# chrischoy/DeepGlobalRegistration

Hardware: AMD Instinct MI355X
Metric: pair registrations/sec (FCGF x2 + 1-NN + 6-D inlier net + gate + weighted Procrustes + SE(3) refinement) (higher is better)
Workload: dtype f32 results via 2 x f16 split operands (3 f16 MFMA products per MAC, f32 accumulate); k = 1 convs, kNN re-evaluation and registration in exact f32, SVD in f64

## Files before the change

### deepglobalregistration_amd/csrc/ctx.hip

```cpp
#include <stdarg.h>
#include <time.h>
#include <string.h>

#include "dgr_internal.h"

static thread_local char g_err[1024] = "";

void dgr_set_error(const char *fmt, ...) {
  va_list ap;
  va_start(ap, fmt);
  vsnprintf(g_err, sizeof(g_err), fmt, ap);
  va_end(ap);
}

extern "C" const char *dgr_last_error(void) { return g_err; }
extern "C" const char *dgr_version(void) { return "dgr_hip 0.4 (gfx950)"; }

static constexpr size_t kAlign = 256;
static constexpr size_t kMinChunk = (size_t)256 << 20;

void *DgrArena::alloc(size_t bytes) {
  bytes = (bytes + kAlign - 1) / kAlign * kAlign;
  if (bytes == 0) bytes = kAlign;
  while (cur < chunks.size()) {
    if (offset + bytes <= chunks[cur].size) {
      void *p = chunks[cur].base + offset;
      offset += bytes;
      used_total += bytes;
      if (used_total > high_water) high_water = used_total;
      return p;
    }
    ++cur;
    offset = 0;
  }
  size_t sz = bytes > kMinChunk ? bytes : kMinChunk;
  size_t have = reserved();
  if (sz < have / 2) sz = have / 2;
  char *base = nullptr;
  hipError_t e = hipMalloc((void **)&base, sz);
  if (e != hipSuccess) {
    dgr_set_error("workspace hipMalloc(%zu MiB) failed: %s", sz >> 20, hipGetErrorString(e));
    return nullptr;
  }
  chunks.push_back({base, sz});
  cur = chunks.size() - 1;
  offset = bytes;
  used_total += bytes;
  if (used_total > high_water) high_water = used_total;
  return base;
}

size_t DgrArena::reserved() const {
  size_t s = 0;
  for (auto &c : chunks) s += c.size;
  return s;
}

int DgrArena::reset() {
  if (chunks.size() > 1) {
    DGR_HIP_CHECK(hipDeviceSynchronize());
    for (auto &c : chunks) DGR_HIP_CHECK(hipFree(c.base));
    chunks.clear();
    size_t want = high_water + high_water / 8 + kAlign;
    char *base = nullptr;
    hipError_t e = hipMalloc((void **)&base, want);
    if (e != hipSuccess) {
      dgr_set_error("workspace hipMalloc(%zu MiB) failed: %s", want >> 20, hipGetErrorString(e));
      return DGR_ENOMEM;
    }
    chunks.push_back({base, want});
  }
  cur = 0;
  offset = 0;
  used_total = 0;
  ++generation;
  return DGR_OK;
}

void DgrArena::release() {
  for (auto &c : chunks) (void)hipFree(c.base);
  chunks.clear();
  cur = offset = 0;
}

hipEvent_t DgrEventPool::next() {
  if (used == ev.size()) {
    hipEvent_t e;
    if (hipEventCreate(&e) != hipSuccess) {
      dgr_set_error("hipEventCreate failed");
      return nullptr;
    }
    ev.push_back(e);
  }
  return ev[used++];
// ... 181 lines not shown
```

### deepglobalregistration_amd/csrc/knn.hip

```cpp
#include "knn_prefilter.h"

template <int C, int QPT>
__global__ void __launch_bounds__(KNN_THREADS)
    knn1_kernel(const float *__restrict__ F0, const float *__restrict__ F1, KnnBatch B, int splits,
                u64 *__restrict__ best, const int32_t *run_flag, const int32_t *__restrict__ qlist,
                const int32_t *qcount, int64_t q_begin) {
  __shared__ __attribute__((aligned(16))) float tile[KNN_TB * C];
  const KnnPair d = B.p[blockIdx.z];
  if (run_flag && run_flag[blockIdx.z] == 0) return;
  F0 += d.q0 * C;
  F1 += d.r0 * C;
  best += d.q0;
  const int64_t N0 = d.n0, N1 = d.n1;
  if (qlist) qlist += d.q0 - q_begin;
  const int64_t n_q = qlist ? (int64_t)qcount[blockIdx.z] : N0;
  if ((int64_t)blockIdx.x * KNN_THREADS * QPT >= n_q) return;
  const int64_t q0 = ((int64_t)blockIdx.x * KNN_THREADS + threadIdx.x) * QPT;
  const int rows_per_split = (int)(((N1 + splits - 1) / splits + KNN_TB - 1) / KNN_TB) * KNN_TB;
  const int64_t j_begin = (int64_t)blockIdx.y * rows_per_split;
  const int64_t j_end = min(N1, j_begin + rows_per_split);
  if (j_begin >= j_end) return;
  float q[QPT][C];
  int64_t qrow[QPT];
#pragma unroll
  for (int u = 0; u < QPT; ++u) {
    const int64_t li = min(q0 + u, n_q - 1);
    const int64_t r = qlist ? (int64_t)qlist[li] : li;
    qrow[u] = r;
#pragma unroll
    for (int c = 0; c < C; c += 4) {
      const float4 v = *reinterpret_cast<const float4 *>(F0 + r * C + c);
      q[u][c] = v.x; q[u][c + 1] = v.y; q[u][c + 2] = v.z; q[u][c + 3] = v.w;
    }
  }
  float bd[QPT];
  int bi[QPT];
#pragma unroll
  for (int u = 0; u < QPT; ++u) { bd[u] = __builtin_inff(); bi[u] = 0x7fffffff; }

  for (int64_t j0 = j_begin; j0 < j_end; j0 += KNN_TB) {
    const int nrows = (int)min((int64_t)KNN_TB, j_end - j0);
    __syncthreads();
    for (int e = threadIdx.x; e < KNN_TB * C / 4; e += KNN_THREADS) {
      const int row = e / (C / 4);
      float4 v = make_float4(0.f, 0.f, 0.f, 0.f);
      if (row < nrows) v = *reinterpret_cast<const float4 *>(F1 + (j0 + row) * C + (e % (C / 4)) * 4);
      *reinterpret_cast<float4 *>(tile + e * 4) = v;
    }
    __syncthreads();
    for (int jj = 0; jj < nrows; ++jj) {
      float d0[QPT], d1[QPT];
#pragma unroll
      for (int u = 0; u < QPT; ++u) { d0[u] = 0.f; d1[u] = 0.f; }
#pragma unroll
      for (int c = 0; c < C; c += 4) {
        const float4 b = *reinterpret_cast<const float4 *>(tile + jj * C + c);
#pragma unroll
        for (int u = 0; u < QPT; ++u) {
          const float e0 = q[u][c] - b.x, e1 = q[u][c + 1] - b.y;
          const float e2 = q[u][c + 2] - b.z, e3 = q[u][c + 3] - b.w;
          d0[u] = fmaf(e0, e0, d0[u]);
          d1[u] = fmaf(e1, e1, d1[u]);
          d0[u] = fmaf(e2, e2, d0[u]);
          d1[u] = fmaf(e3, e3, d1[u]);
        }
      }
#pragma unroll
      for (int u = 0; u < QPT; ++u) {
        const float d = d0[u] + d1[u];
        if (d < bd[u]) { bd[u] = d; bi[u] = (int)(j0 + jj); }
      }
    }
  }
#pragma unroll
  for (int u = 0; u < QPT; ++u) {
    if (q0 + u < n_q && bi[u] != 0x7fffffff)
      atomicMin(best + qrow[u], knn_key(bd[u], bi[u] + (int)d.r0));
  }
}

__global__ void knn1_finish(const u64 *__restrict__ best, KnnBatch B, int squared,
                            int64_t *__restrict__ idx_out, float *__restrict__ dist_out) {
  const KnnPair d = B.p[blockIdx.y];
  const int64_t li = (int64_t)blockIdx.x * blockDim.x + threadIdx.x;
  if (li >= d.n0) return;
  const int64_t i = d.q0 + li;
  const u64 k = best[i];
  idx_out[i] = (k == KNN_KEY_NONE) ? d.r0 : (int64_t)(k & 0xffffffffull);
  if (dist_out) {
    const float d2 = __uint_as_float((unsigned int)(k >> 32));
    dist_out[i] = squared ? d2 : sqrtf(d2 + 1e-7f);
  }
}

template <int C>
static int knn_launch(dgr_ctx *ctx, const float *F0, const float *F1, const KnnBatch &B, u64 *best,
                      const int32_t *run_flag, hipStream_t stream, const int32_t *qlist = nullptr,
                      const int32_t *qcount = nullptr, int64_t q_begin = 0) {
  constexpr int QPT = (C <= 32) ? 4 : 2;
  const dim3 grid = knn_brute_grid(ctx, B, QPT, INT32_MAX);
  knn1_kernel<C, QPT><<<grid, KNN_THREADS, 0, stream>>>(F0, F1, B, (int)grid.y, best, run_flag, qlist, qcount, q_begin);
  DGR_LAUNCH_CHECK();
  return DGR_OK;
}


__global__ void __launch_bounds__(256)
    knn_exact_kernel(const float *__restrict__ F0, const float *__restrict__ F1, const int32_t *__restrict__ cand,
                     const int32_t *__restrict__ cand_cnt, int64_t q_begin, int64_t q_end, u64 *__restrict__ best) {
  const int64_t q = q_begin + (int64_t)blockIdx.x * blockDim.x + threadIdx.x;
  if (q >= q_end) return;
  const int cnt = min(cand_cnt[q - q_begin], KNN_SLOTS);
  if (cnt <= 0) return;
  float a[32];
  knn_load_row<32>(a, F0 + q * 32);
  u64 key = KNN_KEY_NONE;
  for (int slot = 0; slot < cnt; ++slot) {
    const int i = cand[(q - q_begin) * KNN_SLOTS + slot];
    const float d = knn_d2<32>(a, F1 + (int64_t)i * 32);
    if (d < __builtin_inff()) {
      const u64 k2 = knn_key(d, i);
      key = k2 < key ? k2 : key;
    }
  }
  if (key != KNN_KEY_NONE) atomicMin(best + q, key);
}

__global__ void knn_overflow_list(const int32_t *__restrict__ cand_cnt, KnnBatch B, int slots, int64_t q_begin,
                                  int32_t *__restrict__ qlist, int32_t *qcount) {
  const KnnPair d = B.p[blockIdx.y];
  const int64_t q = (int64_t)blockIdx.x * blockDim.x + threadIdx.x;
  if (q < d.n0 && cand_cnt[d.q0 - q_begin + q] > slots)
    qlist[d.q0 - q_begin + atomicAdd(qcount + blockIdx.y, 1)] = (int32_t)q;
}
int knn_list_overflows(const KnnBatch &B, const KnnPlan &P, int slots, hipStream_t stream) {
  dim3 grid((unsigned)dgr_ceil_div(P.n0_max, 256), B.np);
  knn_overflow_list<<<grid, 256, 0, stream>>>(P.cand_cnt, B, slots, P.q_begin, P.qlist, P.qcount);
  DGR_LAUNCH_CHECK();
  return DGR_OK;
}

constexpr int KNN_SCAN_MAX = 64, KNN_SCAN_SPLITS = 16;
__global__ void __launch_bounds__(256)
    knn_query_scan_kernel(const float *__restrict__ F0, const float *__restrict__ F1, KnnBatch B, int64_t q_begin,
                          const int32_t *__restrict__ qlist, const int32_t *__restrict__ qcount,
                          u64 *__restrict__ best) {
  __shared__ u64 wkey[4];
  const KnnPair d = B.p[blockIdx.y];
  const int n_q = qcount[blockIdx.y];
  if (n_q <= 0 || n_q > KNN_SCAN_MAX) return;
  const int per = (d.n1 + KNN_SCAN_SPLITS - 1) / KNN_SCAN_SPLITS;
  const int j_begin = blockIdx.x * per, j_end = min(d.n1, j_begin + per);
  for (int li = 0; li < n_q; ++li) {
    const int64_t q = d.q0 + qlist[d.q0 - q_begin + li];
    float a[32];
    knn_load_row<32>(a, F0 + q * 32);
    u64 key = KNN_KEY_NONE;
    for (int j = j_begin + (int)threadIdx.x; j < j_end; j += 256) {
      const float dd = knn_d2<32>(a, F1 + (d.r0 + j) * 32);
      if (dd < __builtin_inff()) {
        const u64 k2 = knn_key(dd, j + (int)d.r0);
        key = k2 < key ? k2 : key;
      }
    }
#pragma unroll
    for (int s2 = 32; s2 > 0; s2 >>= 1) {
      const u64 o = __shfl_xor(key, s2, 64);
      key = o < key ? o : key;
    }
    if ((threadIdx.x & 63) == 0) wkey[threadIdx.x >> 6] = key;
    __syncthreads();
    if (threadIdx.x == 0) {
      u64 k3 = wkey[0];
      for (int w = 1; w < 4; ++w) k3 = wkey[w] < k3 ? wkey[w] : k3;
      if (k3 != KNN_KEY_NONE) atomicMin(best + q, k3);
    }
    __syncthreads();
  }
}

__global__ void knn_long_list_flags(const int32_t *__restrict__ qcount, int np, int32_t *__restrict__ flags) {
  if ((int)threadIdx.x < np) flags[threadIdx.x] = qcount[threadIdx.x] > KNN_SCAN_MAX;
}

static int knn_prefiltered(dgr_ctx *ctx, const float *F0, const float *F1, KnnBatch B, u64 *best, hipStream_t stream) {
  KnnPlan P;
  DGR_CHECK(knn_prefilter_setup<false>(ctx, F0, F1, B, KNN_SLOTS, stream, &P));
  DGR_CHECK((knn_mfma_launch<false, false>(ctx, B, P, KNN_SUB, KNN_SLOTS, stream)));
  DGR_CHECK((knn_mfma_launch<true, false>(ctx, B, P, 1, KNN_SLOTS, stream)));
  knn_exact_kernel<<<(int)dgr_ceil_div(P.span, 256), 256, 0, stream>>>(F0, F1, P.cand, P.cand_cnt, P.q_begin,
                                                                      P.q_begin + P.span, best);
  DGR_LAUNCH_CHECK();
  DGR_CHECK(knn_list_overflows(B, P, KNN_SLOTS, stream));
  dim3 grid(KNN_SCAN_SPLITS, B.np);
  knn_query_scan_kernel<<<grid, 256, 0, stream>>>(F0, F1, B, P.q_begin, P.qlist, P.qcount, best);
  knn_long_list_flags<<<1, 64, 0, stream>>>(P.qcount, B.np, P.flags);
  DGR_LAUNCH_CHECK();
  DGR_CHECK(knn_launch<32>(ctx, F0, F1, B, best, P.flags, stream, P.qlist, P.qcount, P.q_begin));
  return knn_launch<32>(ctx, F0, F1, B, best, P.fallback, stream);
}

int dgr_knn1_batch_impl(dgr_ctx *ctx, const float *F0, const int64_t *off0, const float *F1, const int64_t *off1,
                        int npairs, int C, int squared, int64_t *idx_out, float *dist_out, hipStream_t stream) {
  return knn_for_each_table(ctx, off0, off1, npairs, 1, true, stream, [&](const KnnBatch &B, u64 *best) -> int {
    DGR_CHECK(knn_dispatch(
        B, C,
        [&](auto width, const KnnBatch &pairs) {
          return knn_launch<decltype(width)::value>(ctx, F0, F1, pairs, best, nullptr, stream);
        },
        [&](const KnnBatch &pairs) { return knn_prefiltered(ctx, F0, F1, pairs, best, stream); }));
    dim3 grid((unsigned)dgr_ceil_div(knn_n0_max(B), 256), B.np);
    knn1_finish<<<grid, 256, 0, stream>>>(best, B, squared, idx_out, dist_out);
    DGR_LAUNCH_CHECK();
    return DGR_OK;
  });
}

int dgr_knn1_impl(dgr_ctx *ctx, const float *F0, int64_t N0, const float *F1, int64_t N1, int C,
                  int squared, int64_t *idx_out, float *dist_out, hipStream_t stream) {
  const int64_t off0[2] = {0, N0}, off1[2] = {0, N1};
  return dgr_knn1_batch_impl(ctx, F0, off0, F1, off1, 1, C, squared, idx_out, dist_out, stream);
}

extern "C" int dgr_knn1_l2(dgr_ctx *ctx, const float *F0, int64_t N0, const float *F1, int64_t N1, int C,
                           int squared, int64_t *idx_out, float *dist_out, dgr_stream stream) {
  const int64_t off0[2] = {0, N0}, off1[2] = {0, N1};
  DGR_CHECK(knn_enter("dgr_knn1_l2", ctx, F0, F1, idx_out, off0, off1, 1));
  return dgr_knn1_impl(ctx, F0, N0, F1, N1, C, squared, idx_out, dist_out, (hipStream_t)stream);
}

extern "C" int dgr_knn1_l2_batch(dgr_ctx *ctx, const float *F0, const int64_t *off0, const float *F1,
                                 const int64_t *off1, int npairs, int C, int squared, int64_t *idx_out,
                                 float *dist_out, dgr_stream stream) {
  DGR_CHECK(knn_enter("dgr_knn1_l2_batch", ctx, F0, F1, idx_out, off0, off1, npairs));
  return dgr_knn1_batch_impl(ctx, F0, off0, F1, off1, npairs, C, squared, idx_out, dist_out, (hipStream_t)stream);
}
```

### deepglobalregistration_amd/csrc/knn_prefilter.h

```cpp
#pragma once
#include "knn_common.h"

typedef __attribute__((ext_vector_type(8))) short bf16x8;
typedef __attribute__((ext_vector_type(16))) float f32x16_t;
constexpr float KNN_TAU_C = 8e-5f;
constexpr int KNN_ST = 4;
constexpr int KNN_SLOTS = 32;
#ifndef DGR_KNN_SUB
#define DGR_KNN_SUB 2
#endif
constexpr int KNN_SUB = DGR_KNN_SUB;

__device__ __forceinline__ unsigned short knn_f2bf(float x) {
  uint32_t u = __float_as_uint(x);
  if ((u & 0x7f800000u) == 0x7f800000u) return (unsigned short)((u >> 16) | ((u & 0xffffu) ? 0x40u : 0u));
  u += 0x7fffu + ((u >> 16) & 1u);
  return (unsigned short)(u >> 16);
}
__device__ __forceinline__ float knn_bf2f(unsigned short h) { return __uint_as_float((uint32_t)h << 16); }
__device__ __forceinline__ uint32_t knn_ord(float f) {
  const uint32_t u = __float_as_uint(f);
  return u ^ ((u >> 31) ? 0xffffffffu : 0x80000000u);
}
__device__ __forceinline__ float knn_unord(uint32_t k) {
  return __uint_as_float(k ^ ((k >> 31) ? 0x80000000u : 0xffffffffu));
}
__device__ __forceinline__ int knn_acc_slot(int e, int h) { return (e & 3) + 8 * (e >> 2) + 4 * h; }

template <bool TOPK>
__device__ __forceinline__ int64_t knn_slot_row(int s, int t, int n_tiles) {
  return (int64_t)(TOPK ? (s + t) & 31 : s) * n_tiles + t;
}
template <bool TOPK>
__global__ void __launch_bounds__(256)
    knn_pack_kernel(const float *__restrict__ F0, const float *__restrict__ F1, KnnBatch B,
                    bf16x8 *__restrict__ Qp, bf16x8 *__restrict__ Rp, float *__restrict__ na, float *__restrict__ nb,
                    uint32_t *__restrict__ nb_max, int32_t *__restrict__ fallback) {
  const int pair = blockIdx.y >> 1, side = blockIdx.y & 1;
  const KnnPair d = B.p[pair];
  const int64_t N = side ? d.n1 : d.n0;
  const int64_t n_pad = (N + 31) / 32 * 32;
  const int64_t t = (int64_t)blockIdx.x * blockDim.x + threadIdx.x;
  int64_t row = t >> 2;
  if (row >= n_pad) return;
  const float *F = side ? F1 + d.r0 * 32 : F0 + d.q0 * 32;
  const float scale = side ? -2.f : 1.f;
  const int64_t prow = row;
  if (side) row = knn_slot_row<TOPK>((int)(prow & 31), (int)(prow >> 5), (int)(n_pad >> 5));
  bf16x8 *packed = side ? Rp + (int64_t)d.rt0 * 256 : Qp + (int64_t)d.qb0 * 256;
  float *norms = side ? nb + (int64_t)d.rt0 * 32 : na + (int64_t)d.qb0 * 32;
  const int g = (int)(t & 1), ch = (int)((t >> 1) & 1);
  bf16x8 hi, lo;
#pragma unroll
  for (int e = 0; e < 8; ++e) { hi[e] = 0; lo[e] = 0; }
  if (row < N) {
    const float *src = F + row * 32 + 16 * ch + 8 * g;
    const float4 v0 = *reinterpret_cast<const float4 *>(src), v1 = *reinterpret_cast<const float4 *>(src + 4);
    const float x[8] = {v0.x, v0.y, v0.z, v0.w, v1.x, v1.y, v1.z, v1.w};
#pragma unroll
    for (int e = 0; e < 8; ++e) {
      if (!(fabsf(x[e]) < 1e18f)) fallback[pair] = 1;
      const unsigned short h = knn_f2bf(x[e]);
      const unsigned short l = knn_f2bf(x[e] - knn_bf2f(h));
      hi[e] = (short)knn_f2bf(knn_bf2f(h) * scale);
      lo[e] = (short)knn_f2bf(knn_bf2f(l) * scale);
    }
  }
  const int64_t tile = prow >> 5;
  const int r = (int)(prow & 31);
  packed[(tile * 4 + ch) * 64 + r + 32 * g] = hi;
  packed[(tile * 4 + 2 + ch) * 64 + r + 32 * g] = lo;
  float n = 0.f;
  if (row < N) {
    const float *src = F + row * 32 + 16 * ch + 8 * g;
#pragma unroll
    for (int e = 0; e < 8; ++e) n = fmaf(src[e], src[e], n);
  }
  n += __shfl_xor(n, 1, 64);
  n += __shfl_xor(n, 2, 64);
  if (g == 0 && ch == 0) {
    if (row >= N) n = side ? __builtin_inff() : 0.f;
    else if (side) atomicMax(nb_max + pair, __float_as_uint(n));
    norms[prow] = n;
  }
}

template <bool PASS2, bool TOPK>
__global__ void __launch_bounds__(256, 2)
    knn_mfma_kernel(const bf16x8 *__restrict__ Qp, const bf16x8 *__restrict__ Rp, const float *__restrict__ nbp,
                    KnnBatch B, int splits, int sub_arg, int64_t q_begin, int64_t span, uint32_t *__restrict__ mt,
                    const float *__restrict__ nap, const uint32_t *__restrict__ nb_max,
                    const float *__restrict__ thr_q, int32_t *__restrict__ cand, int32_t *__restrict__ cand_cnt,
                    int slots_arg) {
  __shared__ bf16x8 sA[2][KNN_ST * 4 * 64];
  __shared__ __attribute__((aligned(16))) float sNb[2][KNN_ST * 32];
  const int sub = TOPK ? sub_arg : KNN_SUB, slots = TOPK ? slots_arg : KNN_SLOTS;
  constexpr int NM = TOPK ? 16 : 1;
  const KnnPair d = B.p[blockIdx.z];
  const int n_qblocks = (d.n0 + 31) >> 5, n_rtiles = (d.n1 + 31) >> 5;
  if ((int)blockIdx.x * 16 >= n_qblocks) return;
  const int64_t N0 = d.n0, N1 = d.n1;
  const bf16x8 *Q = Qp + (int64_t)d.qb0 * 256, *R = Rp + (int64_t)d.rt0 * 256;
  const float *nb = nbp + (int64_t)d.rt0 * 32;
  const int64_t qrow0 = d.q0 - q_begin;
  mt += qrow0;
  cand += qrow0 * slots;
  cand_cnt += qrow0;
  const int tid = threadIdx.x;
  const int lane = tid & 63;
  const int wave = __builtin_amdgcn_readfirstlane(tid >> 6);
  const int h = lane >> 5;
  const int qb0 = (blockIdx.x * 4 + wave) * 4;
  bf16x8 bq[4][4];
  float m[4][NM], thr[4];
#pragma unroll
  for (int u = 0; u < 4; ++u) {
    const int qb = min(qb0 + u, n_qblocks - 1);
#pragma unroll
    for (int f = 0; f < 4; ++f) bq[u][f] = Q[((int64_t)qb * 4 + f) * 64 + lane];
#pragma unroll
    for (int e = 0; e < NM; ++e) m[u][e] = __builtin_inff();
    thr[u] = 0.f;
    if constexpr (PASS2) {
      const int64_t q = (int64_t)qb * 32 + (lane & 31);
      const bool live = q < N0 && qb0 + u < n_qblocks;
      if constexpr (TOPK) {
        thr[u] = live ? thr_q[qrow0 + q] : -__builtin_inff();
      } else {
        const float nmax = __uint_as_float(nb_max[blockIdx.z]);
        thr[u] = live ? knn_unord(mt[q]) + KNN_TAU_C * (nap[(int64_t)d.qb0 * 32 + q] + nmax) : -__builtin_inff();
      }
    }
  }
  const int n_stages = (n_rtiles + KNN_ST - 1) / KNN_ST;
  const int sps = (n_stages + splits - 1) / splits;
  const int s_begin = blockIdx.y * sps, s_end = min(n_stages, s_begin + sps);
  const int step = PASS2 ? 1 : sub;
  const int s_first = PASS2 ? s_begin : s_begin + min((int)(blockIdx.y % sub), max(s_end - s_begin - 1, 0));
  if (s_first >= s_end) return;
  bf16x8 pre[KNN_ST];
  float pre_nb = 0.f;
  auto request = [&](int t0) {
#pragma unroll
    for (int j = 0; j < KNN_ST; ++j) pre[j] = R[(int64_t)min(t0 + j, n_rtiles - 1) * 256 + tid];
    if (tid < KNN_ST * 32) pre_nb = nb[(int64_t)min(t0 + (tid >> 5), n_rtiles - 1) * 32 + (tid & 31)];
  };
  auto deposit = [&](int buf) {
#pragma unroll
    for (int j = 0; j < KNN_ST; ++j) sA[buf][j * 256 + tid] = pre[j];
    if (tid < KNN_ST * 32) sNb[buf][tid] = pre_nb;
  };
  request(s_first * KNN_ST);
  deposit(0);
  __syncthreads();
  int buf = 0;
  for (int st = s_first; st < s_end; st += step) {
    const int t0 = st * KNN_ST;
    if (st + step < s_end) request((st + step) * KNN_ST);
#pragma unroll
    for (int j = 0; j < KNN_ST; ++j) {
      const int t = t0 + j;
      if (t >= n_rtiles) break;
      const bf16x8 a0 = sA[buf][(j * 4 + 0) * 64 + lane], a1 = sA[buf][(j * 4 + 1) * 64 + lane];
      const bf16x8 a2 = sA[buf][(j * 4 + 2) * 64 + lane], a3 = sA[buf][(j * 4 + 3) * 64 + lane];
      f32x16_t c0;
#pragma unroll
      for (int g = 0; g < 4; ++g) {
        const float4 v = *reinterpret_cast<const float4 *>(&sNb[buf][j * 32 + 8 * g + 4 * h]);
        c0[4 * g] = v.x; c0[4 * g + 1] = v.y; c0[4 * g + 2] = v.z; c0[4 * g + 3] = v.w;
      }
      f32x16_t acc[4];
#pragma unroll
      for (int u = 0; u < 4; ++u) acc[u] = __builtin_amdgcn_mfma_f32_32x32x16_bf16(a0, bq[u][0], c0, 0, 0, 0);
#pragma unroll
      for (int u = 0; u < 4; ++u) acc[u] = __builtin_amdgcn_mfma_f32_32x32x16_bf16(a1, bq[u][1], acc[u], 0, 0, 0);
#pragma unroll
      for (int u = 0; u < 4; ++u) acc[u] = __builtin_amdgcn_mfma_f32_32x32x16_bf16(a0, bq[u][2], acc[u], 0, 0, 0);
#pragma unroll
      for (int u = 0; u < 4; ++u) acc[u] = __builtin_amdgcn_mfma_f32_32x32x16_bf16(a1, bq[u][3], acc[u], 0, 0, 0);
#pragma unroll
      for (int u = 0; u < 4; ++u) acc[u] = __builtin_amdgcn_mfma_f32_32x32x16_bf16(a2, bq[u][0], acc[u], 0, 0, 0);
#pragma unroll
      for (int u = 0; u < 4; ++u) acc[u] = __builtin_amdgcn_mfma_f32_32x32x16_bf16(a3, bq[u][1], acc[u], 0, 0, 0);
#pragma unroll
      for (int u = 0; u < 4; ++u) {
        if constexpr (!PASS2 && TOPK) {
#pragma unroll
          for (int e = 0; e < 16; ++e) m[u][e] = fminf(m[u][e], acc[u][e]);
        } else {
          float bm = fminf(fminf(acc[u][0], acc[u][1]), fminf(acc[u][2], acc[u][3]));
#pragma unroll
          for (int e = 4; e < 16; e += 4)
            bm = fminf(bm, fminf(fminf(acc[u][e], acc[u][e + 1]), fminf(acc[u][e + 2], acc[u][e + 3])));
          if constexpr (!PASS2) {
            m[u][0] = fminf(m[u][0], bm);
          } else if (!(bm > thr[u])) {
            const int64_t q = (int64_t)(qb0 + u) * 32 + (lane & 31);
#pragma unroll
            for (int e = 0; e < 16; ++e) {
              const int64_t i = knn_slot_row<TOPK>(knn_acc_slot(e, h), t, n_rtiles);
              if (!(acc[u][e] > thr[u]) && q < N0 && i < N1 && qb0 + u < n_qblocks) {
                const int slot = atomicAdd(cand_cnt + q, 1);
                if (slot < slots) cand[q * slots + slot] = (int32_t)(i + d.r0);
              }
            }
          }
        }
      }
    }
    if (st + step < s_end) deposit(buf ^ 1);
    __syncthreads();
    buf ^= 1;
  }
  if constexpr (!PASS2) {
#pragma unroll
    for (int u = 0; u < 4; ++u) {
      const int64_t q = (int64_t)(qb0 + u) * 32 + (lane & 31);
      const bool live = qb0 + u < n_qblocks && q < N0;
      if constexpr (TOPK) {
        if (live) {
#pragma unroll
          for (int e = 0; e < 16; ++e)
            atomicMin(mt + (int64_t)knn_acc_slot(e, h) * span + q, knn_ord(m[u][e]));
        }
      } else {
        const float mm = fminf(m[u][0], __shfl_xor(m[u][0], 32, 64));
        if (lane < 32 && live) atomicMin(mt + q, knn_ord(mm));
      }
    }
  }
}

struct KnnPlan {
  int64_t q_begin, span, n0_max;
  int qb_max, rt_max;
  int qgroups_all;
  bf16x8 *Qp, *Rp;
  float *na, *nb;
  uint32_t *mt;
  float *thr;
  int32_t *qlist, *cand_cnt, *cand;
  uint32_t *nb_max;
  int32_t *fallback, *qcount, *flags;
};

template <bool TOPK>
inline int knn_prefilter_setup(dgr_ctx *ctx, const float *F0, const float *F1, KnnBatch &B, int slots,
                               hipStream_t stream, KnnPlan *plan) {
  KnnPlan &P = *plan;
  DgrArena &arena = ctx->arena;
  int n_qb = 0, n_rt = 0;
  P.qb_max = P.rt_max = P.qgroups_all = 0;
  for (int p = 0; p < B.np; ++p) {
    KnnPair &d = B.p[p];
    d.qb0 = n_qb;
    d.rt0 = n_rt;
    const int qb = (d.n0 + 31) / 32, rt = (d.n1 + 31) / 32;
    n_qb += qb;
    n_rt += rt;
    P.qb_max = std::max(P.qb_max, qb);
    P.rt_max = std::max(P.rt_max, rt);
    P.qgroups_all += (int)dgr_ceil_div(qb, 16);
  }
  P.n0_max = knn_n0_max(B);
  P.span = knn_query_span(B, &P.q_begin);
  const int64_t n_mt = (TOPK ? 32 : 1) * P.span;
  DGR_ALLOC(P.Qp, arena, bf16x8, (int64_t)n_qb * 256);
  DGR_ALLOC(P.Rp, arena, bf16x8, (int64_t)n_rt * 256);
  DGR_ALLOC(P.na, arena, float, (int64_t)n_qb * 32);
  DGR_ALLOC(P.nb, arena, float, (int64_t)n_rt * 32);
  DGR_ALLOC(P.mt, arena, uint32_t, n_mt);
  P.thr = nullptr;
  if (TOPK) DGR_ALLOC(P.thr, arena, float, P.span);
  DGR_ALLOC(P.qlist, arena, int32_t, P.span);
  DGR_ALLOC(P.cand_cnt, arena, int32_t, P.span + 4 * KNN_MAXP);
  DGR_ALLOC(P.cand, arena, int32_t, P.span * slots);
  int32_t *pair_words = P.cand_cnt + P.span;
  P.nb_max = reinterpret_cast<uint32_t *>(pair_words);
  P.fallback = pair_words + KNN_MAXP;
  P.qcount = pair_words + 2 * KNN_MAXP;
  P.flags = pair_words + 3 * KNN_MAXP;
  DGR_HIP_CHECK(hipMemsetAsync(P.cand_cnt, 0, (size_t)(P.span + 4 * KNN_MAXP) * sizeof(int32_t), stream));
  DGR_HIP_CHECK(hipMemsetAsync(P.mt, 0xff, (size_t)n_mt * sizeof(uint32_t), stream));
  dim3 grid((unsigned)dgr_ceil_div((int64_t)std::max(P.qb_max, P.rt_max) * 32 * 4, 256), 2 * B.np);
  knn_pack_kernel<TOPK><<<grid, 256, 0, stream>>>(F0, F1, B, P.Qp, P.Rp, P.na, P.nb, P.nb_max, P.fallback);
  DGR_LAUNCH_CHECK();
  return DGR_OK;
}

template <bool PASS2, bool TOPK>
inline int knn_mfma_launch(dgr_ctx *ctx, const KnnBatch &B, const KnnPlan &P, int sub, int slots, hipStream_t stream) {
  const auto kernel = knn_mfma_kernel<PASS2, TOPK>;
  static int per_cu = 0;
  if (per_cu == 0) {
    int n = 0;
    DGR_HIP_CHECK(hipOccupancyMaxActiveBlocksPerMultiprocessor(&n, kernel, 256, 0));
    per_cu = n < 1 ? 1 : n;
  }
  const int capacity = ctx->num_cus * per_cu;
  const int stages = (int)dgr_ceil_div(P.rt_max, KNN_ST);
  int splits = 1;
  double best_fill = 0.;
  for (int sp = 1; sp <= std::min(16, std::max(1, stages / sub)); ++sp) {
    const int64_t blocks = (int64_t)P.qgroups_all * sp;
    const double fill = (double)blocks / (double)(dgr_ceil_div(blocks, (int64_t)capacity) * capacity);
    if (fill >= best_fill) { best_fill = fill; splits = sp; }
  }
  dim3 grid((unsigned)dgr_ceil_div(P.qb_max, 16), splits, B.np);
  kernel<<<grid, 256, 0, stream>>>(P.Qp, P.Rp, P.nb, B, splits, sub, P.q_begin, P.span, P.mt, P.na, P.nb_max, P.thr,
                                   P.cand, P.cand_cnt, slots);
  DGR_LAUNCH_CHECK();
  return DGR_OK;
}

int knn_list_overflows(const KnnBatch &B, const KnnPlan &P, int slots, hipStream_t stream);
```

### deepglobalregistration_amd/csrc/knn_topk.hip

```cpp
#include "knn_prefilter.h"

constexpr int KNN_TOPK_SCAN_MAX = 256;
constexpr int KNN_TOPK_MAX_SPLITS = 16;

constexpr int knn_topk_slots(int K) { return K >= 32 ? 512 : 16 * K; }
constexpr int knn_topk_sub(int K) { return K >= 32 ? 1 : 2; }
constexpr int knn_topk_qpt(int C, int K) { return (C + 2 * K) * 4 <= 160 ? 4 : ((C + 2 * K) * 2 <= 160 ? 2 : 1); }

template <int K>
__device__ __forceinline__ void topk_insert(u64 (&L)[K], u64 key) {
  if (key < L[K - 1]) {
#pragma unroll
    for (int i = K - 1; i > 0; --i) {
      const u64 lo = L[i - 1], cur = L[i];
      L[i] = lo > key ? lo : (cur < key ? cur : key);
    }
    L[0] = L[0] < key ? L[0] : key;
  }
}

template <int C, int K, int QPT>
__global__ void __launch_bounds__(KNN_THREADS)
    knn_topk_kernel(const float *__restrict__ F0, const float *__restrict__ F1, KnnBatch B, int splits, int k,
                    int64_t q_begin, int64_t span, u64 *__restrict__ part, const int32_t *__restrict__ run_flag) {
// ... 109 lines not shown
  return DGR_OK;
}

__global__ void __launch_bounds__(256)
    knn_topk_bound(const uint32_t *__restrict__ mt, const float *__restrict__ nap, const uint32_t *__restrict__ nb_max,
                   KnnBatch B, int k, int64_t q_begin, int64_t span, float *__restrict__ thr_q) {
  const KnnPair d = B.p[blockIdx.y];
  const int64_t ql = (int64_t)blockIdx.x * blockDim.x + threadIdx.x;
  if (ql >= d.n0) return;
  const int64_t r = d.q0 - q_begin + ql;
  float v[32];
#pragma unroll
  for (int s = 0; s < 32; ++s) {
    const float x = knn_unord(mt[(int64_t)s * span + r]);
    v[s] = (x == x) ? x : __builtin_inff();
  }
  float U = __builtin_inff();
#pragma unroll
  for (int s = 0; s < 32; ++s) {
    int rank = 0;
#pragma unroll
    for (int t = 0; t < 32; ++t) rank += (v[t] < v[s]) || (v[t] == v[s] && t < s);
    if (rank == k - 1) U = v[s];
  }
  const float nmax = __uint_as_float(nb_max[blockIdx.y]);
  thr_q[r] = U + KNN_TAU_C * (nap[(int64_t)d.qb0 * 32 + ql] + nmax);
}

template <int K>
__global__ void __launch_bounds__(256)
    knn_topk_exact_kernel(const float *__restrict__ F0, const float *__restrict__ F1, const int32_t *__restrict__ cand,
                          const int32_t *__restrict__ cand_cnt, int slots, int k, int64_t q_begin, int64_t q_end,
                          u64 *__restrict__ keys) {
  const int64_t q = q_begin + (int64_t)blockIdx.x * blockDim.x + threadIdx.x;
  if (q >= q_end) return;
  const int cnt = cand_cnt[q - q_begin];
  if (cnt <= 0 || cnt > slots) return;
  float a[32];
  knn_load_row<32>(a, F0 + q * 32);
  u64 L[K];
#pragma unroll
  for (int m = 0; m < K; ++m) L[m] = KNN_KEY_NONE;
  const int32_t *cq = cand + (q - q_begin) * slots;
  for (int s = 0; s < cnt; ++s) {
    const int i = cq[s];
    const float dd = knn_d2<32>(a, F1 + (int64_t)i * 32);
    if (dd < __builtin_inff()) topk_insert<K>(L, knn_key(dd, i));
  }
#pragma unroll
  for (int m = 0; m < K; ++m)
    if (m < k) keys[q * k + m] = L[m];
}

template <int K>
__global__ void __launch_bounds__(256)
    knn_topk_scan_kernel(const float *__restrict__ F0, const float *__restrict__ F1, KnnBatch B, int k, int64_t q_begin,
                         const int32_t *__restrict__ qlist, const int32_t *__restrict__ qcount, u64 *__restrict__ keys) {
  __shared__ u64 wmin[2][4];
  const KnnPair d = B.p[blockIdx.y];
  const int n_q = qcount[blockIdx.y];
  if ((int)blockIdx.x >= n_q || n_q > KNN_TOPK_SCAN_MAX) return;
  const int64_t q = d.q0 + qlist[d.q0 - q_begin + blockIdx.x];
  float a[32];
  knn_load_row<32>(a, F0 + q * 32);
  u64 L[K];
#pragma unroll
  for (int m = 0; m < K; ++m) L[m] = KNN_KEY_NONE;
  for (int j = (int)threadIdx.x; j < d.n1; j += 256) {
    const float dd = knn_d2<32>(a, F1 + (d.r0 + j) * 32);
    if (dd < __builtin_inff()) topk_insert<K>(L, knn_key(dd, j + d.r0));
  }
  for (int r = 0; r < k; ++r) {
    u64 mn = L[0];
#pragma unroll
    for (int s2 = 32; s2 > 0; s2 >>= 1) {
      const u64 o = __shfl_xor(mn, s2, 64);
      mn = o < mn ? o : mn;
    }
    if ((threadIdx.x & 63) == 0) wmin[r & 1][threadIdx.x >> 6] = mn;
    __syncthreads();
    u64 g = wmin[r & 1][0];
#pragma unroll
    for (int w = 1; w < 4; ++w) g = wmin[r & 1][w] < g ? wmin[r & 1][w] : g;
    if (g != KNN_KEY_NONE && L[0] == g) {
#pragma unroll
      for (int m = 0; m < K - 1; ++m) L[m] = L[m + 1];
      L[K - 1] = KNN_KEY_NONE;
    }
    if (threadIdx.x == 0) keys[q * k + r] = g;
  }
}

__global__ void knn_topk_redo_flags(const int32_t *__restrict__ fallback, const int32_t *__restrict__ qcount, int np,
                                    int32_t *__restrict__ flags) {
  if ((int)threadIdx.x < np) flags[threadIdx.x] = fallback[threadIdx.x] != 0 || qcount[threadIdx.x] > KNN_TOPK_SCAN_MAX;
}

template <int K>
static int knn_topk_prefiltered(dgr_ctx *ctx, const float *F0, const float *F1, KnnBatch B, int k, u64 *keys,
                                hipStream_t stream) {
  constexpr int SLOTS = knn_topk_slots(K), SUB = knn_topk_sub(K);
  KnnPlan P;
  DGR_CHECK(knn_prefilter_setup<true>(ctx, F0, F1, B, SLOTS, stream, &P));
  DGR_CHECK((knn_mfma_launch<false, true>(ctx, B, P, SUB, SLOTS, stream)));
  dim3 grid((unsigned)dgr_ceil_div(P.n0_max, 256), B.np);
  knn_topk_bound<<<grid, 256, 0, stream>>>(P.mt, P.na, P.nb_max, B, k, P.q_begin, P.span, P.thr);
// ... 60 lines not shown
```

Baseline: 396.7.

## Replace two-pass 1-NN prefilter with per-stage minima and budgeted stage check

The 1-NN prefiltered search no longer runs a second MFMA pass that collects candidate slots, followed by the exact, overflow-list and query-scan kernels. The first bf16 MFMA pass now also stores a per-stage minimum distance for every query. A new wave-level kernel rechecks in exact f32 only the stages whose minimum falls under each query's threshold, batching those stages in shared memory. Pairs whose flagged-stage count exceeds a budget fall back to the brute-force kernel. This removes one full MFMA pass and several small launches, at the cost of an extra smin buffer and a fallback path that could be slow when the prefilter is weak.

After: 396.6. Within noise of the previous version (-0.0%).

```diff
diff --git a/deepglobalregistration_amd/csrc/ctx.hip b/deepglobalregistration_amd/csrc/ctx.hip
--- a/deepglobalregistration_amd/csrc/ctx.hip
+++ b/deepglobalregistration_amd/csrc/ctx.hip
@@ -40,6 +40,7 @@
   hipError_t e = hipMalloc((void **)&base, sz);
   if (e != hipSuccess) {
     dgr_set_error("workspace hipMalloc(%zu MiB) failed: %s", sz >> 20, hipGetErrorString(e));
+    (void)hipGetLastError();
     return nullptr;
   }
   chunks.push_back({base, sz});
diff --git a/deepglobalregistration_amd/csrc/knn.hip b/deepglobalregistration_amd/csrc/knn.hip
--- a/deepglobalregistration_amd/csrc/knn.hip
+++ b/deepglobalregistration_amd/csrc/knn.hip
@@ -3,8 +3,7 @@
 template <int C, int QPT>
 __global__ void __launch_bounds__(KNN_THREADS)
     knn1_kernel(const float *__restrict__ F0, const float *__restrict__ F1, KnnBatch B, int splits,
-                u64 *__restrict__ best, const int32_t *run_flag, const int32_t *__restrict__ qlist,
-                const int32_t *qcount, int64_t q_begin) {
+                u64 *__restrict__ best, const int32_t *run_flag) {
   __shared__ __attribute__((aligned(16))) float tile[KNN_TB * C];
   const KnnPair d = B.p[blockIdx.z];
   if (run_flag && run_flag[blockIdx.z] == 0) return;
@@ -12,9 +11,7 @@
   F1 += d.r0 * C;
   best += d.q0;
   const int64_t N0 = d.n0, N1 = d.n1;
-  if (qlist) qlist += d.q0 - q_begin;
-  const int64_t n_q = qlist ? (int64_t)qcount[blockIdx.z] : N0;
-  if ((int64_t)blockIdx.x * KNN_THREADS * QPT >= n_q) return;
+  if ((int64_t)blockIdx.x * KNN_THREADS * QPT >= N0) return;
   const int64_t q0 = ((int64_t)blockIdx.x * KNN_THREADS + threadIdx.x) * QPT;
   const int rows_per_split = (int)(((N1 + splits - 1) / splits + KNN_TB - 1) / KNN_TB) * KNN_TB;
   const int64_t j_begin = (int64_t)blockIdx.y * rows_per_split;
@@ -24,8 +21,7 @@
   int64_t qrow[QPT];
 #pragma unroll
   for (int u = 0; u < QPT; ++u) {
-    const int64_t li = min(q0 + u, n_q - 1);
-    const int64_t r = qlist ? (int64_t)qlist[li] : li;
+    const int64_t r = min(q0 + u, N0 - 1);
     qrow[u] = r;
 #pragma unroll
     for (int c = 0; c < C; c += 4) {
@@ -74,7 +70,7 @@
   }
 #pragma unroll
   for (int u = 0; u < QPT; ++u) {
-    if (q0 + u < n_q && bi[u] != 0x7fffffff)
+    if (q0 + u < N0 && bi[u] != 0x7fffffff)
       atomicMin(best + qrow[u], knn_key(bd[u], bi[u] + (int)d.r0));
   }
 }
@@ -95,109 +91,192 @@
 
 template <int C>
 static int knn_launch(dgr_ctx *ctx, const float *F0, const float *F1, const KnnBatch &B, u64 *best,
-                      const int32_t *run_flag, hipStream_t stream, const int32_t *qlist = nullptr,
-                      const int32_t *qcount = nullptr, int64_t q_begin = 0) {
+                      const int32_t *run_flag, hipStream_t stream) {
   constexpr int QPT = (C <= 32) ? 4 : 2;
   const dim3 grid = knn_brute_grid(ctx, B, QPT, INT32_MAX);
-  knn1_kernel<C, QPT><<<grid, KNN_THREADS, 0, stream>>>(F0, F1, B, (int)grid.y, best, run_flag, qlist, qcount, q_begin);
+  knn1_kernel<C, QPT><<<grid, KNN_THREADS, 0, stream>>>(F0, F1, B, (int)grid.y, best, run_flag);
   DGR_LAUNCH_CHECK();
   return DGR_OK;
 }
 
 
-__global__ void __launch_bounds__(256)
-    knn_exact_kernel(const float *__restrict__ F0, const float *__restrict__ F1, const int32_t *__restrict__ cand,
-                     const int32_t *__restrict__ cand_cnt, int64_t q_begin, int64_t q_end, u64 *__restrict__ best) {
-  const int64_t q = q_begin + (int64_t)blockIdx.x * blockDim.x + threadIdx.x;
-  if (q >= q_end) return;
-  const int cnt = min(cand_cnt[q - q_begin], KNN_SLOTS);
-  if (cnt <= 0) return;
-  float a[32];
-  knn_load_row<32>(a, F0 + q * 32);
-  u64 key = KNN_KEY_NONE;
-  for (int slot = 0; slot < cnt; ++slot) {
-    const int i = cand[(q - q_begin) * KNN_SLOTS + slot];
-    const float d = knn_d2<32>(a, F1 + (int64_t)i * 32);
-    if (d < __builtin_inff()) {
-      const u64 k2 = knn_key(d, i);
-      key = k2 < key ? k2 : key;
-    }
-  }
-  if (key != KNN_KEY_NONE) atomicMin(best + q, key);
-}
-
-__global__ void knn_overflow_list(const int32_t *__restrict__ cand_cnt, KnnBatch B, int slots, int64_t q_begin,
-                                  int32_t *__restrict__ qlist, int32_t *qcount) {
+static_assert(KNN_ST == 4, "the stage check deals 16 slots x 4 tiles to the 64 lanes of a wave");
+constexpr int KNN_CHK_LD = 36;
+constexpr int KNN_CHK_LIST = 64;
+constexpr float KNN_STAGE_BUDGET = 0.06f;
+inline float knn_stage_budget() {
+  static const float frac = getenv("DGR_KNN_STAGE_BUDGET") ? (float)atof(getenv("DGR_KNN_STAGE_BUDGET")) : KNN_STAGE_BUDGET;
+  return frac;
+}
+__device__ __forceinline__ u64 knn_budget(const KnnPair &d, int queries, float frac) {
+  const int n_stages = (((d.n1 + 31) >> 5) + KNN_ST - 1) / KNN_ST;
+  return (u64)((float)queries * (2.f + frac * (float)n_stages));
+}
+
+__global__ void __launch_bounds__(64)
+    knn_stage_check_kernel(const float *__restrict__ F0, const float *__restrict__ F1, KnnBatch B, int64_t q_begin,
+                           int64_t span, const uint32_t *__restrict__ mt, const float *__restrict__ nap,
+                           const uint32_t *__restrict__ nb_max, const float *__restrict__ smin, float budget_frac,
+                           u64 *nflag, int32_t *flags, u64 *__restrict__ best) {
+  __shared__ __attribute__((aligned(16))) float rows[64 * KNN_CHK_LD];
+  __shared__ u64 list_mask[KNN_CHK_LIST];
+  __shared__ int list_st[KNN_CHK_LIST];
   const KnnPair d = B.p[blockIdx.y];
-  const int64_t q = (int64_t)blockIdx.x * blockDim.x + threadIdx.x;
-  if (q < d.n0 && cand_cnt[d.q0 - q_begin + q] > slots)
-    qlist[d.q0 - q_begin + atomicAdd(qcount + blockIdx.y, 1)] = (int32_t)q;
-}
-int knn_list_overflows(const KnnBatch &B, const KnnPlan &P, int slots, hipStream_t stream) {
-  dim3 grid((unsigned)dgr_ceil_div(P.n0_max, 256), B.np);
-  knn_overflow_list<<<grid, 256, 0, stream>>>(P.cand_cnt, B, slots, P.q_begin, P.qlist, P.qcount);
-  DGR_LAUNCH_CHECK();
+  const int64_t ql0 = (int64_t)blockIdx.x * 64;
+  if (ql0 >= d.n0) return;
+  const int lane = threadIdx.x;
+  const int64_t N1 = d.n1;
+  const int n_rtiles = (d.n1 + 31) >> 5, n_stages = (n_rtiles + KNN_ST - 1) / KNN_ST;
+  const bool live = ql0 + lane < d.n0;
+  const int64_t ql = min(ql0 + lane, (int64_t)d.n0 - 1);
+  const float na = nap[(int64_t)d.qb0 * 32 + ql];
+  const float thr = knn_unord(mt[d.q0 - q_begin + ql]) + KNN_TAU_C * (na + __uint_as_float(nb_max[blockIdx.y]));
+  const float d_max = thr + na;
+  const float *sm = smin + (d.q0 - q_begin + ql);
+  int cnt = 0;
+  for (int st0 = 0; st0 < n_stages; st0 += 16) {
+    float v[16];
+#pragma unroll
+    for (int k = 0; k < 16; ++k) v[k] = sm[(int64_t)min(st0 + k, n_stages - 1) * span];
+#pragma unroll
+    for (int k = 0; k < 16; ++k) cnt += (live && st0 + k < n_stages && !(v[k] > thr)) ? 1 : 0;
+  }
+#pragma unroll
+  for (int s2 = 32; s2 > 0; s2 >>= 1) cnt += __shfl_xor(cnt, s2, 64);
+  if (cnt == 0) return;
+  u64 before = 0;
+  if (lane == 0) before = atomicAdd(nflag + blockIdx.y, (u64)cnt);
+  before = __shfl(before, 0, 64);
+  if (before + (u64)cnt > knn_budget(d, d.n0, budget_frac) || (u64)cnt > knn_budget(d, 64, budget_frac)) {
+    if (lane == 0) flags[blockIdx.y] = 1;
+    return;
+  }
+
+  const float *F1p = F1 + d.r0 * 32;
+  const int sc = lane >> 5, c4 = lane & 7, jl = (lane >> 3) & 3;
+  int n_list = 0;
+  auto fetch = [&](float4 (&r)[8], int st, int h) {
+    const int t = st * KNN_ST + jl;
+#pragma unroll
+    for (int kk = 0; kk < 8; ++kk) {
+      const int64_t i = knn_slot_row<false>(16 * h + 2 * kk + sc, t, n_rtiles);
+      r[kk] = make_float4(0.f, 0.f, 0.f, 0.f);
+      if (t < n_rtiles && i < N1) r[kk] = *reinterpret_cast<const float4 *>(F1p + i * 32 + c4 * 4);
+    }
+  };
+  auto flush = [&]() {
+    __syncthreads();
+    float4 r[8];
+    fetch(r, list_st[0], 0);
+    for (int n = 0; n < 2 * n_list; ++n) {
+      const int st = __builtin_amdgcn_readfirstlane(list_st[n >> 1]), h = n & 1;
+      const u64 m = list_mask[n >> 1];
+      const u64 mask = ((u64)(uint32_t)__builtin_amdgcn_readfirstlane((int)(m >> 32)) << 32) |
+                       (uint32_t)__builtin_amdgcn_readfirstlane((int)m);
+      float a[32];
+      knn_load_row<32>(a, F0 + (d.q0 + ql0 + __builtin_ctzll(mask)) * 32);
+      __syncthreads();
+#pragma unroll
+      for (int kk = 0; kk < 8; ++kk)
+        *reinterpret_cast<float4 *>(rows + ((2 * kk + sc) * KNN_ST + jl) * KNN_CHK_LD + c4 * 4) = r[kk];
+      __syncthreads();
+      if (n + 1 < 2 * n_list) fetch(r, __builtin_amdgcn_readfirstlane(list_st[(n + 1) >> 1]), (n + 1) & 1);
+      const int t = st * KNN_ST + (lane & 3);
+      const int64_t i = knn_slot_row<false>(16 * h + (lane >> 2), t, n_rtiles);
+      const bool valid = t < n_rtiles && i < N1;
+      for (u64 mk = mask; mk != 0; mk &= mk - 1) {
+        const int b = __builtin_ctzll(mk);
+        if (mk != mask) knn_load_row<32>(a, F0 + (d.q0 + ql0 + b) * 32);
+        const float dd = knn_d2<32>(a, rows + lane * KNN_CHK_LD);
+        const float dm = __shfl(d_max, b, 64);
+        const bool cand = valid && !(dd > dm);
+        const u64 pass = __ballot(cand);
+        if (pass == 0) continue;
+        u64 k2 = cand ? knn_key(dd, i + d.r0) : KNN_KEY_NONE;
+        if (pass & (pass - 1)) {
+#pragma unroll
+          for (int s2 = 32; s2 > 0; s2 >>= 1) {
+            const u64 o = __shfl_xor(k2, s2, 64);
+            k2 = o < k2 ? o : k2;
+          }
+        }
+        if (lane == __builtin_ctzll(pass)) atomicMin(best + d.q0 + ql0 + b, k2);
+      }
+    }
+    __syncthreads();
+    n_list = 0;
+  };
+  for (int st0 = 0; st0 < n_stages; st0 += 8) {
+    float v[8];
+#pragma unroll
+    for (int k = 0; k < 8; ++k) v[k] = sm[(int64_t)min(st0 + k, n_stages - 1) * span];
+#pragma unroll
+    for (int k = 0; k < 8; ++k) {
+      const int st = st0 + k;
+      const u64 mask = __ballot(live && st < n_stages && !(v[k] > thr));
+      if (mask == 0) continue;
+      if (lane == 0) { list_st[n_list] = st; list_mask[n_list] = mask; }
+      if (++n_list == KNN_CHK_LIST) flush();
+    }
+  }
+  if (n_list > 0) flush();
+}
+
+__global__ void knn_redo_flags(const int32_t *__restrict__ fallback, const u64 *__restrict__ nflag, KnnBatch B,
+                               float budget_frac, int32_t *flags) {
+  const int p = threadIdx.x;
+  if (p < B.np) flags[p] = flags[p] != 0 || fallback[p] != 0 || nflag[p] > knn_budget(B.p[p], B.p[p].n0, budget_frac);
+}
+
+static bool knn_trace_on() {
+  static const bool on = getenv("DGR_KNN_TRACE") != nullptr;
+  return on;
+}
+struct KnnTraceClock {
+  hipEvent_t ev[4] = {nullptr, nullptr, nullptr, nullptr};
+  void tick(int i, hipStream_t stream) {
+    if (knn_trace_on() && hipEventCreate(&ev[i]) == hipSuccess) (void)hipEventRecord(ev[i], stream);
+  }
+  ~KnnTraceClock() {
+    for (hipEvent_t e : ev)
+      if (e) (void)hipEventDestroy(e);
+  }
+};
+static int knn_trace(const KnnBatch &B, const KnnPlan &P, const KnnTraceClock &clk, hipStream_t stream) {
+  if (!knn_trace_on()) return DGR_OK;
+  u64 nflag[KNN_MAXP];
+  int32_t words[3 * KNN_MAXP];
+  DGR_HIP_CHECK(hipMemcpyAsync(nflag, P.nflag, sizeof(nflag), hipMemcpyDeviceToHost, stream));
+  DGR_HIP_CHECK(hipMemcpyAsync(words, P.fallback, sizeof(words), hipMemcpyDeviceToHost, stream));
+  DGR_HIP_CHECK(hipStreamSynchronize(stream));
+  for (int p = 0; p < B.np; ++p)
+    fprintf(stderr, "dgr knn1 prefilter: n0=%d n1=%d stages=%d flagged=%llu fallback=%d redo=%d\n", B.p[p].n0, B.p[p].n1,
+            (int)dgr_ceil_div(dgr_ceil_div((int64_t)B.p[p].n1, (int64_t)32), (int64_t)KNN_ST), nflag[p], words[p],
+            words[2 * KNN_MAXP + p]);
+  float ms[3] = {0.f, 0.f, 0.f};
+  for (int i = 0; i < 3; ++i)
+    if (clk.ev[i] && clk.ev[i + 1]) (void)hipEventElapsedTime(&ms[i], clk.ev[i], clk.ev[i + 1]);
+  fprintf(stderr, "dgr knn1 times: pairs=%d pack+mfma=%.3f ms stage_check=%.3f ms redo=%.3f ms\n", B.np, ms[0], ms[1], ms[2]);
   return DGR_OK;
-}
-
-constexpr int KNN_SCAN_MAX = 64, KNN_SCAN_SPLITS = 16;
-__global__ void __launch_bounds__(256)
-    knn_query_scan_kernel(const float *__restrict__ F0, const float *__restrict__ F1, KnnBatch B, int64_t q_begin,
-                          const int32_t *__restrict__ qlist, const int32_t *__restrict__ qcount,
-                          u64 *__restrict__ best) {
-  __shared__ u64 wkey[4];
-  const KnnPair d = B.p[blockIdx.y];
-  const int n_q = qcount[blockIdx.y];
-  if (n_q <= 0 || n_q > KNN_SCAN_MAX) return;
-  const int per = (d.n1 + KNN_SCAN_SPLITS - 1) / KNN_SCAN_SPLITS;
-  const int j_begin = blockIdx.x * per, j_end = min(d.n1, j_begin + per);
-  for (int li = 0; li < n_q; ++li) {
-    const int64_t q = d.q0 + qlist[d.q0 - q_begin + li];
-    float a[32];
-    knn_load_row<32>(a, F0 + q * 32);
-    u64 key = KNN_KEY_NONE;
-    for (int j = j_begin + (int)threadIdx.x; j < j_end; j += 256) {
-      const float dd = knn_d2<32>(a, F1 + (d.r0 + j) * 32);
-      if (dd < __builtin_inff()) {
-        const u64 k2 = knn_key(dd, j + (int)d.r0);
-        key = k2 < key ? k2 : key;
-      }
-    }
-#pragma unroll
-    for (int s2 = 32; s2 > 0; s2 >>= 1) {
-      const u64 o = __shfl_xor(key, s2, 64);
-      key = o < key ? o : key;
-    }
-    if ((threadIdx.x & 63) == 0) wkey[threadIdx.x >> 6] = key;
-    __syncthreads();
-    if (threadIdx.x == 0) {
-      u64 k3 = wkey[0];
-      for (int w = 1; w < 4; ++w) k3 = wkey[w] < k3 ? wkey[w] : k3;
-      if (k3 != KNN_KEY_NONE) atomicMin(best + q, k3);
-    }
-    __syncthreads();
-  }
-}
-
-__global__ void knn_long_list_flags(const int32_t *__restrict__ qcount, int np, int32_t *__restrict__ flags) {
-  if ((int)threadIdx.x < np) flags[threadIdx.x] = qcount[threadIdx.x] > KNN_SCAN_MAX;
 }
 
 static int knn_prefiltered(dgr_ctx *ctx, const float *F0, const float *F1, KnnBatch B, u64 *best, hipStream_t stream) {
   KnnPlan P;
-  DGR_CHECK(knn_prefilter_setup<false>(ctx, F0, F1, B, KNN_SLOTS, stream, &P));
-  DGR_CHECK((knn_mfma_launch<false, false>(ctx, B, P, KNN_SUB, KNN_SLOTS, stream)));
-  DGR_CHECK((knn_mfma_launch<true, false>(ctx, B, P, 1, KNN_SLOTS, stream)));
-  knn_exact_kernel<<<(int)dgr_ceil_div(P.span, 256), 256, 0, stream>>>(F0, F1, P.cand, P.cand_cnt, P.q_begin,
-                                                                      P.q_begin + P.span, best);
+  KnnTraceClock clk;
+  clk.tick(0, stream);
+  DGR_CHECK(knn_prefilter_setup<false>(ctx, F0, F1, B, 0, stream, &P));
+  DGR_CHECK((knn_mfma_launch<false, false>(ctx, B, P, 1, 0, stream)));
+  clk.tick(1, stream);
+  const float budget = knn_stage_budget();
+  dim3 grid((unsigned)dgr_ceil_div(P.n0_max, 64), B.np);
+  knn_stage_check_kernel<<<grid, 64, 0, stream>>>(F0, F1, B, P.q_begin, P.span, P.mt, P.na, P.nb_max, P.smin, budget,
+                                                  P.nflag, P.flags, best);
+  knn_redo_flags<<<1, 64, 0, stream>>>(P.fallback, P.nflag, B, budget, P.flags);
   DGR_LAUNCH_CHECK();
-  DGR_CHECK(knn_list_overflows(B, P, KNN_SLOTS, stream));
-  dim3 grid(KNN_SCAN_SPLITS, B.np);
-  knn_query_scan_kernel<<<grid, 256, 0, stream>>>(F0, F1, B, P.q_begin, P.qlist, P.qcount, best);
-  knn_long_list_flags<<<1, 64, 0, stream>>>(P.qcount, B.np, P.flags);
-  DGR_LAUNCH_CHECK();
-  DGR_CHECK(knn_launch<32>(ctx, F0, F1, B, best, P.flags, stream, P.qlist, P.qcount, P.q_begin));
-  return knn_launch<32>(ctx, F0, F1, B, best, P.fallback, stream);
+  clk.tick(2, stream);
+  DGR_CHECK(knn_launch<32>(ctx, F0, F1, B, best, P.flags, stream));
+  clk.tick(3, stream);
+  return knn_trace(B, P, clk, stream);
 }
 
 int dgr_knn1_batch_impl(dgr_ctx *ctx, const float *F0, const int64_t *off0, const float *F1, const int64_t *off1,
diff --git a/deepglobalregistration_amd/csrc/knn_prefilter.h b/deepglobalregistration_amd/csrc/knn_prefilter.h
--- a/deepglobalregistration_amd/csrc/knn_prefilter.h
+++ b/deepglobalregistration_amd/csrc/knn_prefilter.h
@@ -5,11 +5,6 @@
 typedef __attribute__((ext_vector_type(16))) float f32x16_t;
 constexpr float KNN_TAU_C = 8e-5f;
 constexpr int KNN_ST = 4;
-constexpr int KNN_SLOTS = 32;
-#ifndef DGR_KNN_SUB
-#define DGR_KNN_SUB 2
-#endif
-constexpr int KNN_SUB = DGR_KNN_SUB;
 
 __device__ __forceinline__ unsigned short knn_f2bf(float x) {
   uint32_t u = __float_as_uint(x);
@@ -89,12 +84,12 @@
 __global__ void __launch_bounds__(256, 2)
     knn_mfma_kernel(const bf16x8 *__restrict__ Qp, const bf16x8 *__restrict__ Rp, const float *__restrict__ nbp,
                     KnnBatch B, int splits, int sub_arg, int64_t q_begin, int64_t span, uint32_t *__restrict__ mt,
-                    const float *__restrict__ nap, const uint32_t *__restrict__ nb_max,
-                    const float *__restrict__ thr_q, int32_t *__restrict__ cand, int32_t *__restrict__ cand_cnt,
-                    int slots_arg) {
+                    float *__restrict__ smin, const float *__restrict__ thr_q, int32_t *__restrict__ cand,
+                    int32_t *__restrict__ cand_cnt, int slots) {
+  static_assert(TOPK || !PASS2, "the 1-NN search has one pass");
   __shared__ bf16x8 sA[2][KNN_ST * 4 * 64];
   __shared__ __attribute__((aligned(16))) float sNb[2][KNN_ST * 32];
-  const int sub = TOPK ? sub_arg : KNN_SUB, slots = TOPK ? slots_arg : KNN_SLOTS;
+  const int sub = TOPK ? sub_arg : 1;
   constexpr int NM = TOPK ? 16 : 1;
   const KnnPair d = B.p[blockIdx.z];
   const int n_qblocks = (d.n0 + 31) >> 5, n_rtiles = (d.n1 + 31) >> 5;
@@ -104,8 +99,12 @@
   const float *nb = nbp + (int64_t)d.rt0 * 32;
   const int64_t qrow0 = d.q0 - q_begin;
   mt += qrow0;
-  cand += qrow0 * slots;
-  cand_cnt += qrow0;
+  if constexpr (TOPK) {
+    cand += qrow0 * slots;
+    cand_cnt += qrow0;
+  } else {
+    smin += qrow0;
+  }
   const int tid = threadIdx.x;
   const int lane = tid & 63;
   const int wave = __builtin_amdgcn_readfirstlane(tid >> 6);
@@ -113,6 +112,8 @@
   const int qb0 = (blockIdx.x * 4 + wave) * 4;
   bf16x8 bq[4][4];
   float m[4][NM], thr[4];
+  float ms[4];
+  bool live[4];
 #pragma unroll
   for (int u = 0; u < 4; ++u) {
     const int qb = min(qb0 + u, n_qblocks - 1);
@@ -121,16 +122,10 @@
 #pragma unroll
     for (int e = 0; e < NM; ++e) m[u][e] = __builtin_inff();
     thr[u] = 0.f;
-    if constexpr (PASS2) {
-      const int64_t q = (int64_t)qb * 32 + (lane & 31);
-      const bool live = q < N0 && qb0 + u < n_qblocks;
-      if constexpr (TOPK) {
-        thr[u] = live ? thr_q[qrow0 + q] : -__builtin_inff();
-      } else {
-        const float nmax = __uint_as_float(nb_max[blockIdx.z]);
-        thr[u] = live ? knn_unord(mt[q]) + KNN_TAU_C * (nap[(int64_t)d.qb0 * 32 + q] + nmax) : -__builtin_inff();
-      }
-    }
+    ms[u] = __builtin_inff();
+    const int64_t q = (int64_t)qb * 32 + (lane & 31);
+    live[u] = q < N0 && qb0 + u < n_qblocks;
+    if constexpr (PASS2) thr[u] = live[u] ? thr_q[qrow0 + q] : -__builtin_inff();
   }
   const int n_stages = (n_rtiles + KNN_ST - 1) / KNN_ST;
   const int sps = (n_stages + splits - 1) / splits;
@@ -193,7 +188,7 @@
           for (int e = 4; e < 16; e += 4)
             bm = fminf(bm, fminf(fminf(acc[u][e], acc[u][e + 1]), fminf(acc[u][e + 2], acc[u][e + 3])));
           if constexpr (!PASS2) {
-            m[u][0] = fminf(m[u][0], bm);
+            ms[u] = fminf(ms[u], bm);
           } else if (!(bm > thr[u])) {
             const int64_t q = (int64_t)(qb0 + u) * 32 + (lane & 31);
 #pragma unroll
@@ -208,6 +203,15 @@
         }
       }
     }
+    if constexpr (!TOPK) {
+#pragma unroll
+      for (int u = 0; u < 4; ++u) {
+        const float sm = fminf(ms[u], __shfl_xor(ms[u], 32, 64));
+        if (lane < 32 && live[u]) smin[(int64_t)st * span + (int64_t)(qb0 + u) * 32 + lane] = sm;
+        m[u][0] = fminf(m[u][0], sm);
+        ms[u] = __builtin_inff();
+      }
+    }
     if (st + step < s_end) deposit(buf ^ 1);
     __syncthreads();
     buf ^= 1;
@@ -216,16 +220,14 @@
 #pragma unroll
     for (int u = 0; u < 4; ++u) {
       const int64_t q = (int64_t)(qb0 + u) * 32 + (lane & 31);
-      const bool live = qb0 + u < n_qblocks && q < N0;
       if constexpr (TOPK) {
-        if (live) {
+        if (live[u]) {
 #pragma unroll
           for (int e = 0; e < 16; ++e)
             atomicMin(mt + (int64_t)knn_acc_slot(e, h) * span + q, knn_ord(m[u][e]));
         }
       } else {
-        const float mm = fminf(m[u][0], __shfl_xor(m[u][0], 32, 64));
-        if (lane < 32 && live) atomicMin(mt + q, knn_ord(mm));
+        if (lane < 32 && live[u]) atomicMin(mt + q, knn_ord(m[u][0]));
       }
     }
   }
@@ -238,10 +240,12 @@
   bf16x8 *Qp, *Rp;
   float *na, *nb;
   uint32_t *mt;
+  float *smin;
   float *thr;
   int32_t *qlist, *cand_cnt, *cand;
   uint32_t *nb_max;
   int32_t *fallback, *qcount, *flags;
+  unsigned long long *nflag;
 };
 
 template <bool TOPK>
@@ -270,17 +274,24 @@
   DGR_ALLOC(P.na, arena, float, (int64_t)n_qb * 32);
   DGR_ALLOC(P.nb, arena, float, (int64_t)n_rt * 32);
   DGR_ALLOC(P.mt, arena, uint32_t, n_mt);
-  P.thr = nullptr;
-  if (TOPK) DGR_ALLOC(P.thr, arena, float, P.span);
-  DGR_ALLOC(P.qlist, arena, int32_t, P.span);
-  DGR_ALLOC(P.cand_cnt, arena, int32_t, P.span + 4 * KNN_MAXP);
-  DGR_ALLOC(P.cand, arena, int32_t, P.span * slots);
-  int32_t *pair_words = P.cand_cnt + P.span;
-  P.nb_max = reinterpret_cast<uint32_t *>(pair_words);
-  P.fallback = pair_words + KNN_MAXP;
-  P.qcount = pair_words + 2 * KNN_MAXP;
-  P.flags = pair_words + 3 * KNN_MAXP;
-  DGR_HIP_CHECK(hipMemsetAsync(P.cand_cnt, 0, (size_t)(P.span + 4 * KNN_MAXP) * sizeof(int32_t), stream));
+  P.smin = P.thr = nullptr;
+  P.qlist = P.cand = nullptr;
+  const int64_t n_cnt = TOPK ? (P.span + 1) / 2 * 2 : 0;
+  if (TOPK) {
+    DGR_ALLOC(P.thr, arena, float, P.span);
+    DGR_ALLOC(P.qlist, arena, int32_t, P.span);
+    DGR_ALLOC(P.cand, arena, int32_t, P.span * slots);
+  } else {
+    DGR_ALLOC(P.smin, arena, float, P.span * dgr_ceil_div((int64_t)P.rt_max, (int64_t)KNN_ST));
+  }
+  DGR_ALLOC(P.cand_cnt, arena, int32_t, n_cnt + 6 * KNN_MAXP);
+  int32_t *pair_words = P.cand_cnt + n_cnt;
+  P.nflag = reinterpret_cast<unsigned long long *>(pair_words);
+  P.nb_max = reinterpret_cast<uint32_t *>(pair_words + 2 * KNN_MAXP);
+  P.fallback = pair_words + 3 * KNN_MAXP;
+  P.qcount = pair_words + 4 * KNN_MAXP;
+  P.flags = pair_words + 5 * KNN_MAXP;
+  DGR_HIP_CHECK(hipMemsetAsync(P.cand_cnt, 0, (size_t)(n_cnt + 6 * KNN_MAXP) * sizeof(int32_t), stream));
   DGR_HIP_CHECK(hipMemsetAsync(P.mt, 0xff, (size_t)n_mt * sizeof(uint32_t), stream));
   dim3 grid((unsigned)dgr_ceil_div((int64_t)std::max(P.qb_max, P.rt_max) * 32 * 4, 256), 2 * B.np);
   knn_pack_kernel<TOPK><<<grid, 256, 0, stream>>>(F0, F1, B, P.Qp, P.Rp, P.na, P.nb, P.nb_max, P.fallback);
@@ -307,10 +318,8 @@
     if (fill >= best_fill) { best_fill = fill; splits = sp; }
   }
   dim3 grid((unsigned)dgr_ceil_div(P.qb_max, 16), splits, B.np);
-  kernel<<<grid, 256, 0, stream>>>(P.Qp, P.Rp, P.nb, B, splits, sub, P.q_begin, P.span, P.mt, P.na, P.nb_max, P.thr,
-                                   P.cand, P.cand_cnt, slots);
+  kernel<<<grid, 256, 0, stream>>>(P.Qp, P.Rp, P.nb, B, splits, sub, P.q_begin, P.span, P.mt, P.smin, P.thr, P.cand,
+                                   P.cand_cnt, slots);
   DGR_LAUNCH_CHECK();
   return DGR_OK;
 }
-
-int knn_list_overflows(const KnnBatch &B, const KnnPlan &P, int slots, hipStream_t stream);
diff --git a/deepglobalregistration_amd/csrc/knn_topk.hip b/deepglobalregistration_amd/csrc/knn_topk.hip
--- a/deepglobalregistration_amd/csrc/knn_topk.hip
+++ b/deepglobalregistration_amd/csrc/knn_topk.hip
@@ -185,6 +185,20 @@
     if (m < k) keys[q * k + m] = L[m];
 }
 
+__global__ void knn_overflow_list(const int32_t *__restrict__ cand_cnt, KnnBatch B, int slots, int64_t q_begin,
+                                  int32_t *__restrict__ qlist, int32_t *qcount) {
+  const KnnPair d = B.p[blockIdx.y];
+  const int64_t q = (int64_t)blockIdx.x * blockDim.x + threadIdx.x;
+  if (q < d.n0 && cand_cnt[d.q0 - q_begin + q] > slots)
+    qlist[d.q0 - q_begin + atomicAdd(qcount + blockIdx.y, 1)] = (int32_t)q;
+}
+static int knn_list_overflows(const KnnBatch &B, const KnnPlan &P, int slots, hipStream_t stream) {
+  dim3 grid((unsigned)dgr_ceil_div(P.n0_max, 256), B.np);
+  knn_overflow_list<<<grid, 256, 0, stream>>>(P.cand_cnt, B, slots, P.q_begin, P.qlist, P.qcount);
+  DGR_LAUNCH_CHECK();
+  return DGR_OK;
+}
+
 template <int K>
 __global__ void __launch_bounds__(256)
     knn_topk_scan_kernel(const float *__restrict__ F0, const float *__restrict__ F1, KnnBatch B, int k, int64_t q_begin,
```
